# EarthyScience/EasyHybrid.jl

Hardware: AMD Instinct MI355X
Metric: training samples/sec (higher is better)
Workload: dtype f32; 1 GPU; RbQ10 hybrid, MLP [2,16,16,1] tanh -> rb (sigmoid-scaled), Q10 global, MSE + Adam(0.01), batch=65536 per GPU, fp32 (BASELINE.json configs[1]); global_batch=65536, resident_batches_per_gpu=64, parallelism=dp1, ranks_seen=1, launcher=none, gradient_exchange=none (one GPU)

## Files before the change

### easyhybrid.jl_amd/csrc/eh_api.hip

```cpp
#include <hip/hip_runtime.h>
#include <chrono>

#include <algorithm>
#include <cfloat>
#include <atomic>
#include <cmath>
#include <cstdarg>
#include <cstdio>
#include <cstdlib>
#include <cstring>
#include <memory>
#include <mutex>
#include <string>
#include <thread>
#include <vector>

#include "eh_internal.hpp"
#include "eh_kernels.hpp"
#include "eh_chain.hpp"
#include "eh_lbfgs.hpp"
#include "eh_wide.hpp"
#include "eh_seq.hpp"

std::string g_create_err;
// ... 794 lines not shown
    if (!(h->own_stream = stream_pool_take(h->device))) HIPCHK_C(hipStreamCreateWithFlags(&h->own_stream, hipStreamNonBlocking));
    tick("stream");
    h->stream = h->own_stream;
    for (int vi = 0; vi < arch->nvar; ++vi) HIPCHK_C(arch->var[vi].prepare());
    tick("kernel attributes");
    if (const char* ej = getenv("EH_JIT")) h->jit_on = atoi(ej) != 0;
    if (const char* es = getenv("EH_SPECIALIZE")) h->specialize = atoi(es) != 0;
    if (getenv("EH_NO_AOT_SPEC")) h->aot_spec = false;
    if (d->mech == EH_MECH_PROGRAM) {
        std::vector<unsigned> pb(EH_PROG_HDR + EH_MAX_PROG, 0u);
        pb[0] = (unsigned)d->prog_len; pb[1] = (unsigned)d->prog_n_out;
        for (int o = 0; o < EH_MAX_PROG_OUT; ++o) pb[2 + o] = (unsigned)(o < d->prog_n_out ? d->prog_out[o] : d->prog_out[0]);
        for (int k = 0; k < d->prog_n_const; ++k) memcpy(&pb[8 + k], &d->prog_const[k], sizeof(float));
        for (int i = 0; i < d->prog_len; ++i) pb[EH_PROG_HDR + i] = d->prog_code[i];
        HIPCHK_C(hipMalloc(&h->prog, pb.size() * sizeof(unsigned)));
        HIPCHK_C(hipMemcpy(h->prog, pb.data(), pb.size() * sizeof(unsigned), hipMemcpyHostToDevice));
    }
    const size_t nt = (size_t)n.n_theta;
    HIPCHK_C(hipMalloc(&h->pset, (6 * nt + 4 * EH_MAX_OPT_GROUPS) * sizeof(float)));
    HIPCHK_C(hipMemset(h->pset, 0, (6 * nt + 4 * EH_MAX_OPT_GROUPS) * sizeof(float)));
    for (int k = 0; k < 2; ++k) { h->thb[k] = h->pset + (size_t)k * 3 * nt; h->mb[k] = h->thb[k] + nt; h->vb[k] = h->thb[k] + 2 * nt; }
    h->sc = h->pset + 6 * nt;
    h->bn_on = d->input_batchnorm != 0;
    if (h->bn_on) {
        HIPCHK_C(hipMalloc(&h->bn_part, (32 * 64 + 32) * sizeof(float)));
        HIPCHK_C(hipMalloc(&h->bn_run, 64 * sizeof(float)));
        HIPCHK_C(hipMalloc(&h->bn_shift, 32 * sizeof(float)));
        HIPCHK_C(hipMemset(h->bn_shift, 0, 32 * sizeof(float)));
        HIPCHK_C(hipMalloc(&h->bn_stat, 68 * sizeof(float)));
        HIPCHK_C(hipMemset(h->bn_stat, 0, 68 * sizeof(float)));
        float run0[64];
        for (int p = 0; p < 32; ++p) { run0[p] = 0.0f; run0[32 + p] = 1.0f; }
        HIPCHK_C(hipMemcpy(h->bn_run, run0, sizeof run0, hipMemcpyHostToDevice));
    }
    if (h->bnl) {
        const int tot = h->bnl_maxn;
        int widest = 0;
        for (int l = 0; l < h->l_net[0].nl; ++l) if (h->l_net[0].lbn[l]) widest = std::max(widest, h->l_net[0].out[l]);
        h->bnl_maxn = widest;
        std::vector<float> run0((size_t)tot, 0.0f);
        for (int l = 0; l < h->l_net[0].nl; ++l)
            if (h->l_net[0].lbn[l]) std::fill(run0.begin() + h->bnl_off[l] + h->l_net[0].out[l], run0.begin() + h->bnl_off[l] + 2 * h->l_net[0].out[l], 1.0f);
        HIPCHK_C(hipMalloc(&h->bnl_run, (size_t)tot * sizeof(float)));
        HIPCHK_C(hipMemcpy(h->bnl_run, run0.data(), (size_t)tot * sizeof(float), hipMemcpyHostToDevice));
        HIPCHK_C(hipMalloc(&h->bnl_stat, (size_t)2 * tot * sizeof(float)));
        HIPCHK_C(hipMemset(h->bnl_stat, 0, (size_t)2 * tot * sizeof(float)));
        HIPCHK_C(hipMalloc(&h->bnl_part, (size_t)(EH_BNL_CHUNKS + 1) * 2 * widest * sizeof(float)));
    }
    if (!lform && !seq) {
        HIPCHK_C(hipMalloc(&h->gacc, ((size_t)3 * EH_GSHARDS * h->n_acc + 4) * sizeof(float)));
        HIPCHK_C(hipMemset(h->gacc, 0, ((size_t)3 * EH_GSHARDS * h->n_acc + 4) * sizeof(float)));
        h->ord_soff = (n.n_theta + 3) & ~3;
        h->ord_rs = h->ord_soff + ((h->n_acc - n.n_theta + 3) & ~3);
        const size_t ob = sizeof(unsigned) * 32 * EH_ORD_GROUPS + sizeof(float) * (size_t)2 * (EH_ORD_ROWS + EH_ORD_GROUPS) * h->ord_rs;
        HIPCHK_C(hipMalloc(&h->ord, ob));
        HIPCHK_C(hipMemset(h->ord, 0, ob));
        HIPCHK_C(hipMemsetD32(reinterpret_cast<hipDeviceptr_t>(h->ord + 32 * EH_ORD_GROUPS), (int)EH_ORD_EMPTY, (size_t)2 * EH_ORD_ROWS * h->ord_rs));
        HIPCHK_C(hipHostMalloc((void**)&h->ord_err, sizeof(unsigned), hipHostMallocMapped));
        *h->ord_err = 0u;
    }
    tick("pset / bn / gacc");
    h->slab_rows = lform ? (int)EH_LFORM_ROWS : h->max_blocks;
    HIPCHK_C(hipMalloc(&h->slab, (std::max((size_t)h->slab_rows * std::max(h->n_acc, EH_EVAL_STATS * n.T), (size_t)1 << 20) + 16) * sizeof(float)));
    HIPCHK_C(hipMalloc(&h->gradbuf, (size_t)h->n_acc * sizeof(float)));
    HIPCHK_C(hipMalloc(&h->mombuf, EH_MAX_TARG * EH_EVAL_STATS * sizeof(float)));
    HIPCHK_C(hipMemset(h->mombuf, 0, EH_MAX_TARG * EH_EVAL_STATS * sizeof(float)));
    HIPCHK_C(hipMalloc(&h->tcount, 3 * EH_MAX_TARG * sizeof(float)));
    HIPCHK_C(hipMemset(h->tcount, 0, 3 * EH_MAX_TARG * sizeof(float)));
    HIPCHK_C(hipMalloc(&h->inv_n, EH_TT * EH_MAX_TARG * sizeof(float)));
    HIPCHK_C(hipMemset(h->inv_n, 0, EH_TT * EH_MAX_TARG * sizeof(float)));
    HIPCHK_C(hipMemset(h->gradbuf, 0, (size_t)h->n_acc * sizeof(float)));
    tick("slab + small buffers");
    if (seq) {
        std::vector<unsigned char> wf((size_t)n.n_theta, 0);
        const int* o = h->seq_off;
        std::fill(wf.begin() + o[EH_SEQ_WIN], wf.begin() + o[EH_SEQ_BIN], (unsigned char)1);
        std::fill(wf.begin() + o[EH_SEQ_WHD], wf.begin() + o[EH_SEQ_BHD], (unsigned char)1);
        std::fill(wf.begin() + o[EH_SEQ_WOUT], wf.begin() + o[EH_SEQ_BOUT], (unsigned char)1);
        HIPCHK_C(hipMalloc(&h->wflag, wf.size()));
        HIPCHK_C(hipMemcpy(h->wflag, wf.data(), wf.size(), hipMemcpyHostToDevice));
    }
    else if (!lform) { if (int rc = build_maps(h, true)) { g_create_err = h->err; eh_destroy(h); return rc; } }
    else {
        std::vector<unsigned char> wf((size_t)n.n_theta, 0);
        for (int k = 0; k < h->l_nnets; ++k)
            for (int l = 0; l < h->l_net[k].nl; ++l)
                if (!h->l_net[k].lbn[l]) std::fill(wf.begin() + h->l_net[k].woff[l], wf.begin() + h->l_net[k].boff[l], (unsigned char)1);
        HIPCHK_C(hipMalloc(&h->wflag, wf.size()));
        HIPCHK_C(hipMemcpy(h->wflag, wf.data(), wf.size(), hipMemcpyHostToDevice));
    }
    tick("maps");
    {
        std::vector<float> img0((size_t)arch->img_floats, 0.0f);
        for (int j = 0; j < d->n_params; ++j) {
            if (d->param_kind[j] == EH_PAR_FIXED) img0[arch->phi_off + EH_IMG_PHI + j] = d->param_default[j];
            img0[arch->phi_off + EH_IMG_LO + j] = d->param_lower[j];
            img0[arch->phi_off + EH_IMG_SC + j] = d->param_upper[j] - d->param_lower[j];
        }
        for (int p = 0; p < 32; ++p) { img0[arch->phi_off + EH_IMG_BNM + p] = 0.0f; img0[arch->phi_off + EH_IMG_BNR + p] = d->input_batchnorm ? 1.0f / std::sqrt(1.0f + EH_BN_EPS) : 1.0f; }
        for (int k = 0; k < (lform ? 0 : n_nets); ++k)
            for (int l = net_d[k]; l < nl; ++l)
                for (int i = 0; i < net_w[k][l]; ++i)
                    img0[arch->wh_off + (size_t)(l - 1) * arch->hp * arch->sh + (size_t)(h->net_r0[k][l] + i) * arch->sh + h->net_r0[k][l - 1] + i] = 1.0f;
        auto put_int = [&](int slot, int v) { memcpy(&img0[arch->phi_off + slot], &v, sizeof(int)); };
        if (!lform && !seq) {
            for (int l = 0; l <= d->n_hidden; ++l) { put_int(EH_IMG_WOFF + l, lw_off[l]); put_int(EH_IMG_BOFF + l, lb_off[l]); }
            for (int l = 0; l < d->n_hidden; ++l) put_int(EH_IMG_WIDTH + l, tot_w[l]);
// ... 707 lines not shown
    if (!spec_lookup(h) && jit_wanted(h, EH_MODE_TRAIN)) {
        eh_handle_s::JitEntry* je = jit_entry(const_cast<eh_handle*>(h));
        if (je && (!je->verified || !je->k.fn[EH_MODE_TRAIN_MULTI])) return false;
    }
    return true;
}
static int do_fused_multi(eh_handle* h, const EhSplit& sp, const int* idx, long long first, long long batch, long long end, int nsteps, float* loss_slots) {
    if (h->pending && h->pend_ord) FLUSH(h);
    EhStepArgs a = eh_step_args(h, sp, idx, first, std::min(batch, end - first));
    a.image = h->image; a.slab = h->slab; a.n_acc = h->n_acc; a.inv_n = nullptr; a.rmap = h->rmap; a.stamps = h->stamps;
    EhFused& z = a.fz;
    z.gacc = h->gacc; z.pset = h->pset; z.imap = h->imap; z.loss_slot = h->pending_loss;
    z.gslot = (int)(h->gstep % 3); z.cur = h->cur; z.sc_sel = h->sc_sel; z.pending = h->pending ? 1 : 0; z.opt = h->opt; z.agg_a = h->img.agg_a;
    a.p2p = nullptr; a.p2p_seq = 0u;
    if (int rc = eh_bn_prepare(h, sp, idx, first, a.count, true, &a)) return rc;
    a.ms_nsteps = nsteps; a.ms_batch = (int)batch; a.ms_end = end; a.ms_loss = loss_slots;
    HIPCHK(h, step_launch(h, EH_MODE_TRAIN_MULTI, 1, &a));
    h->cur ^= 1; h->sc_sel ^= 1;
    h->gstep += 1;
    h->pending = false;
    h->pending_loss = nullptr;
    return EH_OK;
}

static int launch_chain(eh_handle* h, bool raw, float* sc_in, float* sc_out, float* loss_slot) {
    static const int one_env = getenv("EH_CHAIN_ONE") ? atoi(getenv("EH_CHAIN_ONE")) : -1;
    const int nt = h->net.n_theta;
    const bool l2 = raw && (h->img.l2c != 0.0f || h->img.l2w);
    const unsigned tp = raw ? two_pass_mask(h->net) : 0u;
    const EhChainSrc src{raw ? 1 : 0, h->net.loss, h->net.T, tp, tp ? h->inv_n : nullptr, l2 ? h->l2val : nullptr};
    unsigned long long* ctr = reinterpret_cast<unsigned long long*>(h->chain_part + EH_CHAIN_PARTS);
    if (h->chain.i_norm < 0) {
        hipLaunchKernelGGL(eh_chain_apply_kernel<false>, dim3((nt + 255) / 256), dim3(256), 0, h->stream, h->gradbuf, nt, TH(h), MM(h), VV(h), sc_in, sc_out, h->opt,
                           h->chain, src, h->img, h->chain_part, 0, loss_slot, ctr);
    } else if (nt <= (one_env >= 0 ? one_env : (int)EH_CHAIN_ONE_MAX)) {
        hipLaunchKernelGGL(eh_chain_apply_kernel<true>, dim3(1), dim3(256), 0, h->stream, h->gradbuf, nt, TH(h), MM(h), VV(h), sc_in, sc_out, h->opt,
                           h->chain, src, h->img, h->chain_part, 0, loss_slot, ctr);
    } else {
        const int nb = std::min<int>(EH_CHAIN_PARTS, (nt + 1023) / 1024);
        hipLaunchKernelGGL(eh_chain_norm_kernel, dim3(nb), dim3(256), 0, h->stream, h->gradbuf, nt, TH(h), h->chain, src, h->img, h->chain_part);
        HIPCHK(h, hipGetLastError());
        hipLaunchKernelGGL(eh_chain_apply_kernel<false>, dim3((nt + 255) / 256), dim3(256), 0, h->stream, h->gradbuf, nt, TH(h), MM(h), VV(h), sc_in, sc_out, h->opt,
                           h->chain, src, h->img, h->chain_part, nb, loss_slot, ctr);
    }
    HIPCHK(h, hipGetLastError());
    return EH_OK;
}

static bool ord_ok(const eh_handle* h, int grid) {
    static const int cw_env = getenv("EH_REDUCE_CW") ? atoi(getenv("EH_REDUCE_CW")) : 0;
    if (!h->fused || !h->fused_det || !h->ord || grid <= 1 || grid > (int)EH_ORD_ROWS || h->chain.n || h->drop_on) return false;
    if (h->lform || h->arch->wide || h->p2p_on || h->net.T != 1 || h->net.mech == EH_MECH_PROGRAM || h->net.loss == EH_LOSS_PROGRAM || h->act == EH_ACT_PER_NET) return false;
    if (h->img.l2c != 0.0f || h->img.l2w || two_pass_mask(h->net) || h->dp_weights || h->dp_moments) return false;
    return h->n_acc < 8192 && h->ord_rs <= h->arch->img_floats && (cw_env == 0 || cw_env == 16);
}

int eh_do_step(eh_handle* h, const EhSplit& sp, const int* idx, long long first, long long count, bool apply, bool raw, float* loss_slot) {
    const EhNet& net = h->net;
    EhProf prof;
    if (int rc = prof_begin(h, &prof)) return rc;
    int grid = 1;
    const int deferred = (net.T == 1 && !raw) ? 1 : 0;
    const unsigned tp_mask = two_pass_mask(net);
    const bool moment_loss = tp_mask != 0;
    const bool l2 = (h->img.l2c != 0.0f || h->img.l2w) && !raw;
    float* sc_in = h->sc + 2 * h->sc_sel;
    float* sc_out = h->sc + 2 * (h->sc_sel ^ 1);
    EhLApply lap{};
    h->l_apply = nullptr; h->l_applied = false;
    const bool chained = apply && h->chain.n != 0;
    if (h->lform && apply && deferred && !l2 && !moment_loss && net.loss != EH_LOSS_PROGRAM) {
        lap.theta = TH(h); lap.m = MM(h); lap.v = VV(h); lap.sc_in = sc_in; lap.sc_out = sc_out; lap.o = h->opt; lap.loss_slot = loss_slot; lap.gradbuf = h->gradbuf;
        lap.im = h->img; lap.loss_kind = h->net.loss; lap.n_theta = net.n_theta; lap.g_off = net.g_off;
        if (chained) {
            HIPCHK(h, hipMemsetAsync(h->gradbuf, 0, (size_t)net.n_theta * sizeof(float), h->stream));
            lap.theta = h->gradbuf;
            lap.o = EhOpt{EH_OPT_DESCENT, -1.0f, 1.0f, 1.0f, 0.0f, 0.0f, nullptr};
            lap.im.g_off = net.n_theta; lap.im.imap = nullptr;
        }
        h->l_apply = &lap;
    }
    int rc = launch_train_kernel(h, sp, idx, first, count, &grid, apply);
    h->l_apply = nullptr;
    if (rc) return rc;
    if (h->drop_on && apply) h->drop_step++;
    const bool mid = prof.on && !prof.burst;
    if (mid) HIPCHK(h, hipEventRecord(h->ev[h->ev_used + 1], h->stream));
    if (h->l_applied) {
        h->l_applied = false;
        if (chained) {
            if (int rcc = launch_chain(h, false, sc_in, sc_out, nullptr)) return rcc;
        }
        h->sc_sel ^= 1;
        return prof_end(h, prof, mid);
    }
    if (l2) {
        hipLaunchKernelGGL(eh_weight_l2_kernel, dim3(1), dim3(256), 0, h->stream, TH(h), h->img, h->l2val);
        HIPCHK(h, hipGetLastError());
    }
    static const int cw_env = getenv("EH_REDUCE_CW") ? atoi(getenv("EH_REDUCE_CW")) : 0;
    const bool big = cw_env ? cw_env == 64 : h->n_acc >= 8192;
    const bool tall = cw_env ? cw_env == 256 : (h->lform && grid <= (int)EH_LFORM_ROWS && h->n_acc >= 16384);
    static const bool nc1 = getenv("EH_REDUCE_NC1") != nullptr;
    const bool tall4 = tall && !nc1;
    const int rgrid = tall4 ? (h->n_acc + 1023) / 1024 : tall ? (h->n_acc + 255) / 256 : big ? (h->n_acc + 63) / 64 : (h->n_acc + 15) / 16;
#define EH_REDUCE_GO(AP, ...)                                                                                                                       \
// ... 967 lines not shown
```

### easyhybrid.jl_amd/csrc/eh_device.hpp

```cpp
#pragma once
#ifndef __HIPCC_RTC__
#include <hip/hip_runtime.h>
#include <stdint.h>
#endif

#include "easyhybrid_hip.h"

#define EH_BN_SELF_MAX 512
#define EH_EVAL_STATS 8

typedef float f32x4 __attribute__((ext_vector_type(4)));

enum { EH_MODE_TRAIN = 0, EH_MODE_EVAL = 1, EH_MODE_TRAIN_P2P = 2, EH_MODE_TRAIN_MULTI = 3, EH_MODE_TRAIN_ORD = 4 };

struct EhNet {
    int P, K, G, T, F;
    int n_theta, g_off;
    int scale_nn, mech, n_par;
    int loss;
    int n_out;
    unsigned targ_out;
    unsigned par_kind;
    unsigned par_idx;
    unsigned forc_col;
// ... 32 lines not shown
    } else if (o.rule == EH_OPT_RMSPROP) {
        v = o.b1 * v + (1.0f - o.b1) * (g * g);
        th -= g * (o.lr / (sqrtf(v) + o.eps));
    } else {
        th -= o.lr * g;
    }
}

template <class PB>
__device__ __forceinline__ void eh_opt_update_at(const EhOpt& o, PB bt, long long i, float g, float bt1, float bt2, float& th, float& m, float& v) {
    if (o.tab == nullptr) { eh_opt_update(o, g, bt1, bt2, th, m, v); return; }
    const int k = o.tab->gid[i];
    eh_opt_update(o.tab->r[k], g, bt[4 * k], bt[4 * k + 1], th, m, v);
}
template <class PI, class PO>
__device__ __forceinline__ void eh_opt_advance_groups(const EhOptTab* tab, PI bt_in, PO bt_out, bool upd) {
    const int n = tab->n;
    for (int k = 0; k < n; ++k) {
        const float p1 = bt_in[4 * k], p2 = bt_in[4 * k + 1];
        bt_out[4 * k] = upd ? p1 * tab->r[k].b1 : p1;
        bt_out[4 * k + 1] = upd ? p2 * tab->r[k].b2 : p2;
    }
}

__device__ __forceinline__ void eh_loss_finish(int kind, float S, float n, float Sy, float Syy, float& scale, float& loss, float agg = 1.0f) {
    if (!(n > 0.0f)) { scale = 0.0f; loss = __builtin_nanf(""); return; }
    if (kind == EH_LOSS_RMSE) {
        loss = sqrtf(S / n);
        scale = 1.0f / (2.0f * n * loss);
    } else if (kind == EH_LOSS_NSELOSS) {
        const float D = Syy - Sy * Sy / n;
        loss = S / D;
        scale = 1.0f / D;
    } else {
        scale = 1.0f / n;
        loss = S * scale;
    }
    if (agg != 1.0f) { scale *= agg; loss *= agg; }
}

#define EH_GSHARDS 8

struct EhP2P {
    unsigned long long* peer_recv[EH_GSHARDS];
    float* stage;
    unsigned* counter;
    int* err;
    int world, rank;
    int mode;
};

template <int CTRL> __device__ __forceinline__ float eh_dpp(float v);
enum { EH_ORD_GROUPS = 16, EH_ORD_ROWS = 256 };
struct EhOrd {
    float* rows;
    float* grows;
    unsigned* cnt;
    unsigned* err;
    int rs, soff;
    int slot;
    int prev_grid;
};
#define EH_ORD_EMPTY 0x7FA5A5A5u
#define EH_ORD_DEADLINE_TICKS 200000000ull
enum { EH_ORD_ST_TAIL = 32, EH_ORD_ST_PRO = EH_ORD_ST_TAIL + 10 * EH_ORD_GROUPS, EH_STAMP_WORDS = 256 };
#ifdef EH_STAMPS
#define EH_ORD_TICK(ts, p)                                                                            \
    do {                                                                                               \
        __builtin_amdgcn_sched_barrier(0);                                                             \
        ts[2 * (p)] = __builtin_readcyclecounter(); ts[2 * (p) + 1] = wall_clock64();                  \
        __builtin_amdgcn_sched_barrier(0);                                                             \
    } while (0)
#else
#define EH_ORD_TICK(ts, p)
#endif
__device__ __forceinline__ int eh_ord_pos(int e, int nth, int soff) { return e < nth ? e : soff + (e - nth); }
#ifdef EH_AB_ORD_PARENT
__device__ __forceinline__ int eh_ord_scalar_row(int lane) { return lane; }
__device__ __forceinline__ f32x4 eh_ord_scalar_fold(const EhOrd& o, int lane, const f32x4 (&v)[4]) {
    float w[4][4];
#pragma unroll
    for (int j = 0; j < 4; ++j)
#pragma unroll
        for (int k = 0; k < 4; ++k) {
            float c = 0.0f;
            if (lane + 64 * j < o.prev_grid) c += v[j][k];
#pragma unroll
            for (int off = 32; off >= 1; off >>= 1) c += __shfl_xor(c, off, 64);
            w[j][k] = c;
        }
    f32x4 t;
#pragma unroll
    for (int k = 0; k < 4; ++k) t[k] = (w[0][k] + w[1][k]) + (w[2][k] + w[3][k]);
    return t;
}
#else
__device__ __forceinline__ int eh_ord_scalar_row(int lane) { return 4 * (lane & ~15) + (lane & 15); }
__device__ __forceinline__ f32x4 eh_ord_scalar_fold(const EhOrd& o, int lane, const f32x4 (&v)[4]) {
    const int r0 = eh_ord_scalar_row(lane);
    f32x4 t;
#pragma unroll
    for (int k = 0; k < 4; ++k) {
        float c[4];
#pragma unroll
        for (int j = 0; j < 4; ++j) {
            c[j] = 0.0f;
            if (r0 + 16 * j < o.prev_grid) c[j] += v[j][k];
        }
        float s = (c[0] + c[2]) + (c[1] + c[3]);
        s += eh_dpp<0x128>(s);
        s += eh_dpp<0x124>(s);
        s += eh_dpp<0x4E>(s);
        s += eh_dpp<0xB1>(s);
        const int si = __builtin_bit_cast(int, s);
        const float w0 = __builtin_bit_cast(float, __builtin_amdgcn_readlane(si, 0)), w1 = __builtin_bit_cast(float, __builtin_amdgcn_readlane(si, 16)),
                    w2 = __builtin_bit_cast(float, __builtin_amdgcn_readlane(si, 32)), w3 = __builtin_bit_cast(float, __builtin_amdgcn_readlane(si, 48));
        t[k] = (w0 + w1) + (w2 + w3);
    }
    return t;
}
#endif
__device__ __forceinline__ void eh_ord_scalar_loads(const EhOrd& o, int lane, f32x4 (&v)[4]) {
    const float* const R = o.rows + (long long)(o.slot ^ 1) * EH_ORD_ROWS * o.rs + o.soff;
    const int r0 = eh_ord_scalar_row(lane);
#pragma unroll
    for (int j = 0; j < 4; ++j) {
        const int r = r0 + 16 * j;
        v[j] = r < o.prev_grid ? *(const f32x4*)(R + (long long)r * o.rs) : f32x4{0.0f, 0.0f, 0.0f, 0.0f};
    }
}
__device__ __forceinline__ void eh_ord_group_loads(const EhOrd& o, int idx, float (&g)[EH_ORD_GROUPS]) {
    const float* const G = o.grows + (long long)(o.slot ^ 1) * EH_ORD_GROUPS * o.rs + idx;
#pragma unroll
    for (int k = 0; k < EH_ORD_GROUPS; ++k) g[k] = k < o.prev_grid ? G[(long long)k * o.rs] : 0.0f;
}
__device__ __forceinline__ float eh_ord_group_fold(const float (&g)[EH_ORD_GROUPS]) {
    float t = 0.0f;
#pragma unroll
    for (int k = 0; k < EH_ORD_GROUPS; ++k) t += g[k];
    return t;
}
typedef unsigned u32x4_ord __attribute__((ext_vector_type(4)));
__device__ __forceinline__ __amdgpu_buffer_rsrc_t eh_ord_rsrc(const float* base, int nfloats) {
    return __builtin_amdgcn_make_buffer_rsrc(const_cast<float*>(base), (short)0, 4 * nfloats, 0x00020000);
}
__device__ __forceinline__ f32x4 eh_ord_ld16(__amdgpu_buffer_rsrc_t r, int off) { return __builtin_bit_cast(f32x4, __builtin_amdgcn_raw_buffer_load_b128(r, off, 0, 16)); }
__device__ __forceinline__ void eh_ord_st16(__amdgpu_buffer_rsrc_t r, int off, f32x4 v) { __builtin_amdgcn_raw_buffer_store_b128(__builtin_bit_cast(u32x4_ord, v), r, off, 0, 16); }
enum { EH_ORD_OOB = 0x7FFFFFF0 };
__device__ __forceinline__ void eh_ord_reset(const EhOrd& o, int b, int nblk, int tid, int nthr) {
    const __amdgpu_buffer_rsrc_t rr = eh_ord_rsrc(o.rows, 2 * EH_ORD_ROWS * o.rs);
    const float e = __uint_as_float(EH_ORD_EMPTY);
    const f32x4 ev = {e, e, e, e};
    const int nv = o.soff >> 2;
    for (int r = b; r < o.prev_grid; r += nblk)
        for (int v = tid; v < nv; v += nthr) eh_ord_st16(rr, 4 * (((o.slot ^ 1) * EH_ORD_ROWS + r) * o.rs) + 16 * v, ev);
}
__device__ __forceinline__ void eh_ord_publish(const EhOrd& o, int nth, int tid, int nthr, const float* row, float* flag, unsigned long long* st) {
#ifdef EH_STAMPS
    unsigned long long ts[10];
#endif
    EH_ORD_TICK(ts, 0);
    const unsigned gi = blockIdx.x % EH_ORD_GROUPS, gsz = (gridDim.x - gi + EH_ORD_GROUPS - 1) / EH_ORD_GROUPS;
    const __amdgpu_buffer_rsrc_t rr = eh_ord_rsrc(o.rows, 2 * EH_ORD_ROWS * o.rs);
    const int nv = (nth + 3) >> 2;
#ifdef EH_AB_ORD_PARENT
    asm volatile("s_waitcnt vmcnt(0)" ::: "memory");
#endif
    __syncthreads();
    if (__builtin_amdgcn_readfirstlane(tid >> 6) == 0) {
        const int rb = 4 * ((o.slot * EH_ORD_ROWS + (int)blockIdx.x) * o.rs);
        for (int v = tid; v <= nv; v += 64) {
            const int w = v < nv ? 4 * v : o.soff;
            eh_ord_st16(rr, rb + 4 * w, *(const f32x4*)&row[w]);
        }
        EH_ORD_TICK(ts, 1);
        if (tid == 0) {
            unsigned* const gc = o.cnt + 32 * gi;
            const bool last = __hip_atomic_fetch_add(gc, 1u, __ATOMIC_RELAXED, __HIP_MEMORY_SCOPE_AGENT) == gsz - 1;
            if (last) __hip_atomic_store(gc, 0u, __ATOMIC_RELAXED, __HIP_MEMORY_SCOPE_AGENT);
            flag[0] = last ? 1.0f : 0.0f;
        }
    }
    __syncthreads();
    EH_ORD_TICK(ts, 2);
    if (flag[0] == 0.0f) return;
    constexpr int NK = EH_ORD_ROWS / EH_ORD_GROUPS;
    const int kown = blockIdx.x / EH_ORD_GROUPS;
    const int rb = 4 * ((o.slot * EH_ORD_ROWS + (int)gi) * o.rs), rk = 4 * EH_ORD_GROUPS * o.rs;
    const __amdgpu_buffer_rsrc_t gr = eh_ord_rsrc(o.grows, 2 * EH_ORD_GROUPS * o.rs);
    const int gb = 4 * ((o.slot * EH_ORD_GROUPS + (int)gi) * o.rs);
    for (int v = tid; v < nv; v += nthr) {
        f32x4 r[NK];
#pragma unroll
        for (int k = 0; k < NK; ++k) r[k] = eh_ord_ld16(rr, ((unsigned)k < gsz && k != kown) ? rb + k * rk + 16 * v : (int)EH_ORD_OOB);
        const f32x4 own = *(const f32x4*)&row[4 * v];
        auto fold = [&]() {
            f32x4 s = {0.0f, 0.0f, 0.0f, 0.0f};
#pragma unroll
            for (int k = 0; k < NK; ++k) s += k == kown ? own : r[k];
            return s;
        };
        f32x4 s = fold();
        bool nan = false;
#pragma unroll
        for (int j = 0; j < 4; ++j) nan = nan || (4 * v + j < nth && s[j] != s[j]);
        if (nan) {
            auto empty = [&](int k) {
                bool e = false;
#pragma unroll
                for (int j = 0; j < 4; ++j) e = e || (4 * v + j < nth && __float_as_uint(r[k][j]) == EH_ORD_EMPTY);
                return e;
            };
            bool in = true;
#pragma unroll
            for (int k = 0; k < NK; ++k) in = in && !empty(k);
            if (!in) {
                const unsigned long long t0 = wall_clock64();
                bool late = false;
                s = f32x4{0.0f, 0.0f, 0.0f, 0.0f};
#pragma unroll 1
                for (int k = 0; k < NK; ++k) {
                    f32x4 q = own;
                    if (k != kown) {
                        const int off = (unsigned)k < gsz ? rb + k * rk + 16 * v : (int)EH_ORD_OOB;
                        auto empty_q = [&]() {
                            bool e = false;
#pragma unroll
                            for (int j = 0; j < 4; ++j) e = e || (4 * v + j < nth && __float_as_uint(q[j]) == EH_ORD_EMPTY);
                            return e;
                        };
                        q = eh_ord_ld16(rr, off);
                        while (!late && empty_q()) {
                            if (wall_clock64() - t0 > EH_ORD_DEADLINE_TICKS) { __hip_atomic_store(o.err, 1u, __ATOMIC_RELAXED, __HIP_MEMORY_SCOPE_SYSTEM); late = true; break; }
                            __builtin_amdgcn_s_sleep(1);
                            q = eh_ord_ld16(rr, off);
                        }
                    }
                    s += q;
                }
            }
        }
        eh_ord_st16(gr, gb + 16 * v, s);
    }
// ... 698 lines not shown
    int nx_glb = 0;
    bool nx_live = false;
    auto fetch_idx = [&](int tile) {
        const int n_loc = tile * MT + lane;
        nx_live = (tile < ntiles) && (lane < MT) && (n_loc < count);
        nx_glb = nx_live ? (a.idx ? a.idx[first + n_loc] : first + n_loc) : 0;
    };
    auto fetch_rec_into = [&](EhRec<NX4>& dst) {
        const bool live = nx_live;
        const float* const rec = a.recs + (long long)nx_glb * a.C;
        if ((a.C & 3) == 0) {
#pragma unroll
            for (int q = 0; q < NX4; ++q) dst.x[q] = (live && 4 * q < net.P) ? *(const f32x4*)(rec + 4 * q) : f32x4{0, 0, 0, 0};
        } else {
#pragma unroll
            for (int q = 0; q < NX4; ++q)
#pragma unroll
                for (int e = 0; e < 4; ++e) dst.x[q][e] = (live && 4 * q + e < net.P) ? rec[4 * q + e] : 0.0f;
        }
#pragma unroll
        for (int f = 0; f < EH_MAX_FORC; ++f) dst.frc[f] = (fCol[f] >= 0 && live) ? rec[fCol[f]] : 0.0f;
#pragma unroll
        for (int t = 0; t < EH_MAX_TARG; ++t) dst.y[t] = (tOn[t] != 0.0f && live) ? rec[tcol0 + t] : __builtin_nanf("");
    };
    auto fetch_rec = [&]() { fetch_rec_into(nx); };
    auto fetch = [&](int tile) { fetch_idx(tile); fetch_rec(); };
    const bool carried = carry && carry->valid;
    bool rec_pending = false;
    if (carried) { nx = carry->rec; nx_live = carry->live; }
    else {
        fetch_idx((int)blockIdx.x * NW + wave);
        rec_pending = a.idx != nullptr;
        if (!rec_pending) fetch_rec();
    }
    bool pf_issued = false;

    EH_STAMP(0);
    const bool fusedm = TRAIN && a.fz.gacc != nullptr;
    float f_th = 0.0f, f_m = 0.0f, f_v = 0.0f, f_g = 0.0f, f_cnt = 0.0f, f_sse = 0.0f, f_sy = 0.0f, f_syy = 0.0f, f_bt1 = 0.0f, f_bt2 = 0.0f;
    int f_map = 0;
    int f_rcode = 0;
    if constexpr (TRAIN) f_rcode = (a.rmap && tid < a.n_acc) ? a.rmap[tid] : 0;
    float f_rm = 0.0f, f_rv = 0.0f;
    if ((a.bn_part || a.bn_nblk == -1) && a.bn_update && blockIdx.x == 0 && tid < net.P) { f_rm = a.bn_run[tid]; f_rv = a.bn_run[32 + tid]; }
    const bool deferred_upd = fusedm && !(a.ms_direct && a.ms_keep);
    const int px_mode = P2PM ? a.p2pv.mode : 0, px_rank = P2PM ? a.p2pv.rank : 0, px_world = P2PM ? a.p2pv.world : 1;
    const unsigned long long* const px_recv = P2PM ? a.p2pv.peer_recv[px_rank] + (long long)((a.fz.gslot + 2) % 3) * EH_GSHARDS * a.n_acc : nullptr;
    const float* const px_stage = P2PM ? a.p2pv.stage : nullptr;
    float px_own[5] = {0.0f, 0.0f, 0.0f, 0.0f, 0.0f};
    const bool own_direct = deferred_upd && a.fz.pending && (!P2PM || px_mode == 1);
    float f_sv = 0.0f;
    float f_gs[EH_GSHARDS] = {0.0f, 0.0f, 0.0f, 0.0f, 0.0f, 0.0f, 0.0f, 0.0f};
    float o_g[ORDM ? EH_ORD_GROUPS : 1];
    f32x4 o_sv[ORDM ? 4 : 1];
    if constexpr (ORDM) {
#pragma unroll
        for (int k = 0; k < EH_ORD_GROUPS; ++k) o_g[k] = 0.0f;
#pragma unroll
        for (int j = 0; j < 4; ++j) o_sv[j] = f32x4{0.0f, 0.0f, 0.0f, 0.0f};
    }
    if (deferred_upd) {
        const EhFused& z = a.fz;
        const float* const g_prev = (P2PM ? px_stage : z.gacc) + ((z.gslot + 2) % 3) * (EH_GSHARDS * a.n_acc);
        const float* const pin = z.pset + z.cur * 3 * net.n_theta;
        if constexpr (ORDM) { if (own_direct && wave == 0) eh_ord_scalar_loads(a.ord, lane, o_sv); }
        else { if (own_direct && lane < 40) f_sv = g_prev[(lane & 7) * a.n_acc + net.n_theta + (lane >> 3)]; }
        const float* const sc_in = z.pset + 6 * net.n_theta + 2 * z.sc_sel;
        f_bt1 = sc_in[0]; f_bt2 = sc_in[1];
        if (tid < net.n_theta) {
            f_th = pin[tid]; f_m = pin[net.n_theta + tid]; f_v = pin[2 * net.n_theta + tid];
            f_map = tid < net.g_off ? z.imap[tid] : 0;
            if (own_direct) {
                if constexpr (ORDM) eh_ord_group_loads(a.ord, tid, o_g);
                else {
#pragma unroll
                    for (int sh = 0; sh < EH_GSHARDS; ++sh) f_gs[sh] = g_prev[sh * a.n_acc + tid];
                }
            }
        }
    }
    EH_STAMP_PRO(2);
    float* const px_T = eh_px_table<P2PM || ORDM>();
    const int px_nmain = net.n_theta < NTHR ? net.n_theta : NTHR;
    const unsigned px_seq = a.p2p_seq - 1u;
    const unsigned long long px_none = (unsigned long long)px_seq << 32;
    unsigned long long px_w[P2PM ? EH_GSHARDS : 1], px_s[P2PM ? EH_GSHARDS : 1];
    const int px_k = tid - (NTHR - 8);
    const bool px_sc = px_k >= 0 && px_k < (net.T > 3 ? 5 : 4);
    auto px_request = [&]() {
#pragma unroll
        for (int sh = 0; sh < (P2PM ? EH_GSHARDS : 1); ++sh) {
            px_w[sh] = px_none; px_s[sh] = px_none;
            if (sh < px_world && !(px_mode == 1 && sh == px_rank)) {
                const unsigned long long* const q = px_recv + (long long)sh * a.n_acc;
                if (tid < px_nmain) px_w[sh] = __hip_atomic_load(q + tid, __ATOMIC_RELAXED, __HIP_MEMORY_SCOPE_SYSTEM);
                if (px_sc) px_s[sh] = __hip_atomic_load(q + net.n_theta + px_k, __ATOMIC_RELAXED, __HIP_MEMORY_SCOPE_SYSTEM);
            }
        }
    };
    if constexpr (P2PM) {
        if (fusedm && a.fz.pending && px_mode == 1 && px_world > 1 && blockIdx.x == 0) eh_p2p_fold_store(&a.p2pv, (a.fz.gslot + 2) % 3, px_seq, a.n_acc, tid, NTHR, true);
        if (fusedm && a.fz.pending) px_request();
    }
    EH_STAMP_PRO(3);
    if (!a.ms_keep) {
        constexpr int NI = (G::IMG_FLOATS / 4 + NTHR - 1) / NTHR, NIB = NI < 16 ? NI : 16;
        for (int e0 = 4 * tid; e0 < G::IMG_FLOATS; e0 += 4 * NTHR * NIB) {
            f32x4 tmp[NIB];
#pragma unroll
            for (int u = 0; u < NIB; ++u) {
                const int e = e0 + 4 * NTHR * u;
                tmp[u] = e < G::IMG_FLOATS ? *(const f32x4*)&a.image[e] : f32x4{0, 0, 0, 0};
            }
            if (rec_pending) { fetch_rec(); rec_pending = false; }
#pragma unroll
            for (int u = 0; u < NIB; ++u) {
                const int e = e0 + 4 * NTHR * u;
                if (e < G::IMG_FLOATS) *(f32x4*)&wl[e] = tmp[u];
            }
        }
    }
    if (rec_pending) fetch_rec();
    if (ORDM && own_direct) {
        if constexpr (ORDM) {
#ifdef EH_STAMPS
            if (a.stamps && blockIdx.x == 0 && tid == 0) { unsigned long long ts[4]; EH_ORD_TICK(ts, 0); a.stamps[EH_ORD_ST_PRO] = ts[0]; a.stamps[EH_ORD_ST_PRO + 1] = ts[1]; }
#endif
            f_g = eh_ord_group_fold(o_g);
            if (wave == 0) {
                const f32x4 t = eh_ord_scalar_fold(a.ord, lane, o_sv);
                if (lane == 0) *(f32x4*)px_T = t;
#ifdef EH_STAMPS
                if (a.stamps && blockIdx.x == 0 && tid == 0) { unsigned long long ts[4]; EH_ORD_TICK(ts, 1); a.stamps[EH_ORD_ST_PRO + 2] = ts[2]; a.stamps[EH_ORD_ST_PRO + 3] = ts[3]; }
#endif
            }
        }
    } else if (own_direct) {
        f_g = eh_fold8(f_gs[0], f_gs[1], f_gs[2], f_gs[3], f_gs[4], f_gs[5], f_gs[6], f_gs[7]);
        const int svi = __builtin_bit_cast(int, eh_fold8_lanes(f_sv));
        const float S0 = __builtin_bit_cast(float, __builtin_amdgcn_readlane(svi, 0)), S1 = __builtin_bit_cast(float, __builtin_amdgcn_readlane(svi, 8)),
                    S2 = __builtin_bit_cast(float, __builtin_amdgcn_readlane(svi, 16)), S3 = __builtin_bit_cast(float, __builtin_amdgcn_readlane(svi, 24)),
                    S4 = __builtin_bit_cast(float, __builtin_amdgcn_readlane(svi, 32));
        if constexpr (P2PM) { px_own[0] = S0; px_own[1] = S1; px_own[2] = S2; px_own[3] = S3; px_own[4] = S4; }
        else {
            f_sse = S0; f_cnt = S1 + (net.T > 1 ? S2 : 0.0f) + (net.T > 2 ? S3 : 0.0f) + (net.T > 3 ? S4 : 0.0f); f_sy = S2; f_syy = S3;
        }
    }
    EH_STAMP_PRO(4);
    if constexpr (P2PM) {
        if (fusedm && a.fz.pending) {
            {
                unsigned long long t0 = 0;
                bool timing = false;
                while (true) {
                    bool all = true;
#pragma unroll
                    for (int sh = 0; sh < EH_GSHARDS; ++sh)
                        if (sh < px_world) all = all && ((unsigned)(px_w[sh] >> 32) == px_seq) && ((unsigned)(px_s[sh] >> 32) == px_seq);
                    if (all) break;
                    if (__hip_atomic_load(a.p2pv.err, __ATOMIC_RELAXED, __HIP_MEMORY_SCOPE_AGENT)) break;
                    if (!timing) { t0 = wall_clock64(); timing = true; }
                    else if (wall_clock64() - t0 > EH_P2P_DEADLINE_TICKS) { __hip_atomic_store(a.p2pv.err, 1, __ATOMIC_RELAXED, __HIP_MEMORY_SCOPE_AGENT); break; }
                    __builtin_amdgcn_s_sleep(2);
                    px_request();
                }
            }
            EH_STAMP_PRO(11);
            const bool own1 = px_mode == 1;
            const float own_g = f_g;
            const float own_s = px_k == 0 ? px_own[0] : px_k == 1 ? px_own[1] : px_k == 2 ? px_own[2] : px_k == 3 ? px_own[3] : px_own[4];
            float fs = 0.0f;
            f_g = 0.0f;
#pragma unroll
            for (int sh = 0; sh < EH_GSHARDS; ++sh)
                if (sh < px_world) {
                    const bool own = own1 && sh == px_rank;
                    f_g += own ? own_g : ((unsigned)(px_w[sh] >> 32) == px_seq) ? __uint_as_float((unsigned)px_w[sh]) : 0.0f;
                    fs += own ? own_s : ((unsigned)(px_s[sh] >> 32) == px_seq) ? __uint_as_float((unsigned)px_s[sh]) : 0.0f;
                }
            if (px_k >= 0) px_T[px_k] = fs;
            EH_STAMP_PRO(12);
            __syncthreads();
            EH_STAMP_PRO(13);
            {
                const f32x4 t4 = *(const f32x4*)px_T;
                f_sse = t4[0];
// ... 1095 lines not shown
```

### easyhybrid.jl_amd/csrc/eh_kernels.hpp

```cpp
#pragma once
#include "eh_internal.hpp"

__global__ __launch_bounds__(256) void eh_weight_l2_kernel(const float* theta, EhImg im, float* out) {
    __shared__ float red[4];
    float s = 0.0f;
    if (im.l2w) {
        for (int i = threadIdx.x; i < im.n_theta; i += 256) { const float w = theta[i]; s = fmaf(im.l2w[i] * w, w, s); }
    } else {
        for (int i = threadIdx.x; i < im.g_off; i += 256)
            if (eh_is_weight(im, i)) { const float w = theta[i]; s += w * w; }
    }
#pragma unroll
    for (int o = 32; o >= 1; o >>= 1) s += __shfl_xor(s, o, 64);
    if ((threadIdx.x & 63) == 0) red[threadIdx.x >> 6] = s;
    __syncthreads();
    if (threadIdx.x == 0) *out = im.l2s * (im.l2w ? 1.0f : im.l2c) * ((red[0] + red[1]) + (red[2] + red[3]));
}

__global__ void eh_image_kernel(const float* theta, int n_theta, EhImg im) {
    const int idx = blockIdx.x * blockDim.x + threadIdx.x;
    if (idx < n_theta) eh_image_store(im, idx, theta[idx]);
}


// ... 234 lines not shown
        float got[6 * EH_GSHARDS];
        eh_ll_issue(ad, seq, w);
        eh_ll_finish(p2p, ad, seq, w, got);
        float s1 = 0.0f, s2 = 0.0f, s3 = 0.0f, s4 = 0.0f;
#pragma unroll
        for (int sh = 0; sh < EH_GSHARDS; ++sh) {
            const bool me = own_direct && sh == p2p->rank;
            sse += me ? ownv[0] : got[6 * sh]; s1 += me ? ownv[1] : got[6 * sh + 1]; s2 += me ? ownv[2] : got[6 * sh + 2];
            s3 += me ? ownv[3] : got[6 * sh + 3]; s4 += me ? ownv[4] : got[6 * sh + 4]; gs_p2p += me ? ownv[5] : got[6 * sh + 5];
        }
        cnt = s1 + (T > 1 ? s2 : 0.0f) + (T > 2 ? s3 : 0.0f) + (T > 3 ? s4 : 0.0f); sy = s2; syy = s3;
    } else {
        static_assert(EH_GSHARDS == 8, "eh_fold8");
        float S[5] = {0.0f, 0.0f, 0.0f, 0.0f, 0.0f};
#pragma unroll
        for (int k = 0; k < 5; ++k) {
            if (k == 4 && T <= 3) continue;
            const float* q = g_prev + n_theta + k;
            S[k] = eh_fold8(q[0], q[n_acc], q[2 * n_acc], q[3 * n_acc], q[4 * n_acc], q[5 * n_acc], q[6 * n_acc], q[7 * n_acc]);
        }
        sse = S[0]; cnt = S[1] + (T > 1 ? S[2] : 0.0f) + (T > 2 ? S[3] : 0.0f) + (T > 3 ? S[4] : 0.0f); sy = S[2]; syy = S[3];
    }
    float inv = 0.0f, lossv = 0.0f;
    if (T == 1) eh_loss_finish(loss_kind, sse, cnt, sy, syy, inv, lossv, im.agg_a);
    else { inv = cnt > 0.0f ? 1.0f : 0.0f; lossv = cnt > 0.0f ? sse : __builtin_nanf(""); }
    float th = th0;
    if (own && cnt > 0.0f) {
        const float gs = p2p ? gs_p2p : eh_fold8(gsv[0], gsv[1], gsv[2], gsv[3], gsv[4], gsv[5], gsv[6], gsv[7]);
        float mm = mm0, vv = vv0;
        eh_opt_update_at(o, sc_in, idx, gs * inv, sc0, sc1, th, mm, vv);
        theta[idx] = th; m[idx] = mm; v[idx] = vv;
    }
    if (own) {
        if (idx < im.g_off) { if (mp0 >= 0) im.image[mp0] = th; }
        else eh_image_store(im, idx, th);
    }
    if (idx == 0) {
        if (o.tab) eh_opt_advance_groups(o.tab, sc_in, sc_out, cnt > 0.0f);
        else {
            sc_out[0] = cnt > 0.0f ? sc0 * o.b1 : sc0;
            sc_out[1] = cnt > 0.0f ? sc1 * o.b2 : sc1;
        }
        if (loss_slot) *loss_slot = lossv;
    }
}

__global__ __launch_bounds__(256) void eh_ord_flush_kernel(const EhOrd o, int n_theta, float* theta, float* m, float* v, const float* sc_in, float* sc_out,
                                                           EhOpt op, float* loss_slot, EhImg im, int loss_kind) {
    eh_ord_reset(o, blockIdx.x, gridDim.x, threadIdx.x, 256);
    if ((int)blockIdx.x * 256 >= n_theta) return;
    const int idx = blockIdx.x * 256 + threadIdx.x, lane = threadIdx.x & 63;
    const bool own = idx < n_theta;
    float gv[EH_ORD_GROUPS];
    f32x4 sv[4];
    eh_ord_group_loads(o, own ? idx : 0, gv);
    eh_ord_scalar_loads(o, lane, sv);
    float th = 0.0f, mm = 0.0f, vv = 0.0f;
    int mp = -1;
    if (own) { th = theta[idx]; mm = m[idx]; vv = v[idx]; if (idx < im.g_off && im.imap) mp = im.imap[idx]; }
    const float bt1 = sc_in[0], bt2 = sc_in[1];
    const f32x4 t = eh_ord_scalar_fold(o, lane, sv);
    float inv = 1.0f, lossv = 0.0f;
    eh_loss_finish(loss_kind, t[0], t[1], t[2], t[3], inv, lossv, im.agg_a);
    const bool upd = t[1] > 0.0f;
    if (own && upd) {
        eh_opt_update_at(op, sc_in, idx, eh_ord_group_fold(gv) * inv, bt1, bt2, th, mm, vv);
        theta[idx] = th; m[idx] = mm; v[idx] = vv;
    }
    if (own) {
        if (idx < im.g_off) { if (mp >= 0) im.image[mp] = th; }
        else eh_image_store(im, idx, th);
    }
    if (idx == 0) {
        if (op.tab) eh_opt_advance_groups(op.tab, sc_in, sc_out, upd);
        else {
            sc_out[0] = upd ? bt1 * op.b1 : bt1;
            sc_out[1] = upd ? bt2 * op.b2 : bt2;
        }
        if (loss_slot) *loss_slot = upd ? lossv + 0.0f : __builtin_nanf("");
    }
}

__device__ __forceinline__ bool eh_kind_two_pass(unsigned kind, int T) {
    return (kind >= (unsigned)EH_LOSS_PEARSONLOSS && kind <= (unsigned)EH_LOSS_PBKGELOSS) || (kind == (unsigned)EH_LOSS_RMSE && T > 1);
}
__global__ __launch_bounds__(64) void eh_moment_centre_kernel(const float* slab, int nblk, int T, unsigned loss_t, EhShift4 shift, float* tt) {
    __shared__ double tot[EH_EVAL_STATS];
    const int tid = threadIdx.x, t = blockIdx.x;
    if (!eh_kind_two_pass((loss_t >> (4 * t)) & 15u, T)) return;
    if (tid < EH_EVAL_STATS) {
        double s = 0.0;
        for (int b = 0; b < nblk; ++b) s += (double)slab[(b * T + t) * EH_EVAL_STATS + tid];
        tot[tid] = s;
    }
    __syncthreads();
    if (tid == 0) tt[EH_TT * t + 1] = tot[3] > 0.0 ? (float)((double)shift.c[t] + tot[4] / tot[3]) : shift.c[t];
}
__global__ __launch_bounds__(64) void eh_moment_coef_kernel(const float* slab, int nblk, int T, unsigned loss_t, EhShift4 shift4, float* tt_all, float agg_a) {
    __shared__ double tot[EH_EVAL_STATS];
    const int tid = threadIdx.x, t = blockIdx.x;
    const int kind = (int)((loss_t >> (4 * t)) & 15u);
    if (!eh_kind_two_pass((unsigned)kind, T)) return;
    float* const out = tt_all + EH_TT * t;
    const float shift = shift4.c[t];
    if (tid < EH_EVAL_STATS) {
        double s = 0.0;
        for (int b = 0; b < nblk; ++b) s += (double)slab[(b * T + t) * EH_EVAL_STATS + tid];
// ... 190 lines not shown
```

Before: 6.377 billion samples/s.

## Pre-reduce ordered loss scalars per group into a partial buffer

Adds a small per-group partial buffer where the last wave of each group-reducing block pre-folds the four loss scalars across its rows, waiting on empty sentinels if needed. The next step's prologue and flush kernel then load one f32x4 per lane from this buffer instead of four row loads, and fold with DPP and readlane. The work can run on the last wave when the parameter count leaves it idle. It adds a spin-wait path and restricts the ordered mode to layouts with exactly four scalar slots.

```diff
diff --git a/easyhybrid.jl_amd/csrc/eh_api.hip b/easyhybrid.jl_amd/csrc/eh_api.hip
--- a/easyhybrid.jl_amd/csrc/eh_api.hip
+++ b/easyhybrid.jl_amd/csrc/eh_api.hip
@@ -870,7 +870,7 @@
         HIPCHK_C(hipMemset(h->gacc, 0, ((size_t)3 * EH_GSHARDS * h->n_acc + 4) * sizeof(float)));
         h->ord_soff = (n.n_theta + 3) & ~3;
         h->ord_rs = h->ord_soff + ((h->n_acc - n.n_theta + 3) & ~3);
-        const size_t ob = sizeof(unsigned) * 32 * EH_ORD_GROUPS + sizeof(float) * (size_t)2 * (EH_ORD_ROWS + EH_ORD_GROUPS) * h->ord_rs;
+        const size_t ob = sizeof(unsigned) * 32 * EH_ORD_GROUPS + sizeof(float) * ((size_t)2 * (EH_ORD_ROWS + EH_ORD_GROUPS) * h->ord_rs + 2 * EH_ORD_PART);
         HIPCHK_C(hipMalloc(&h->ord, ob));
         HIPCHK_C(hipMemset(h->ord, 0, ob));
         HIPCHK_C(hipMemsetD32(reinterpret_cast<hipDeviceptr_t>(h->ord + 32 * EH_ORD_GROUPS), (int)EH_ORD_EMPTY, (size_t)2 * EH_ORD_ROWS * h->ord_rs));
@@ -1684,6 +1684,7 @@
     if (!h->fused || !h->fused_det || !h->ord || grid <= 1 || grid > (int)EH_ORD_ROWS || h->chain.n || h->drop_on) return false;
     if (h->lform || h->arch->wide || h->p2p_on || h->net.T != 1 || h->net.mech == EH_MECH_PROGRAM || h->net.loss == EH_LOSS_PROGRAM || h->act == EH_ACT_PER_NET) return false;
     if (h->img.l2c != 0.0f || h->img.l2w || two_pass_mask(h->net) || h->dp_weights || h->dp_moments) return false;
+    if (h->n_acc != h->net.n_theta + 4 || h->ord_rs != h->ord_soff + 4) return false;
     return h->n_acc < 8192 && h->ord_rs <= h->arch->img_floats && (cw_env == 0 || cw_env == 16);
 }
 
diff --git a/easyhybrid.jl_amd/csrc/eh_device.hpp b/easyhybrid.jl_amd/csrc/eh_device.hpp
--- a/easyhybrid.jl_amd/csrc/eh_device.hpp
+++ b/easyhybrid.jl_amd/csrc/eh_device.hpp
@@ -108,6 +108,10 @@
 
 template <int CTRL> __device__ __forceinline__ float eh_dpp(float v);
 enum { EH_ORD_GROUPS = 16, EH_ORD_ROWS = 256 };
+enum { EH_ORD_PART = 4 * EH_ORD_GROUPS * 4 };
+#if defined(EH_AB_ORD_PARENT) && !defined(EH_AB_ORD_ROW_SCALARS)
+#define EH_AB_ORD_ROW_SCALARS
+#endif
 struct EhOrd {
     float* rows;
     float* grows;
@@ -131,6 +135,30 @@
 #define EH_ORD_TICK(ts, p)
 #endif
 __device__ __forceinline__ int eh_ord_pos(int e, int nth, int soff) { return e < nth ? e : soff + (e - nth); }
+#ifndef EH_AB_ORD_ROW_SCALARS
+enum { EH_ORD_NSV = 1 };
+__device__ __forceinline__ f32x4 eh_ord_scalar_fold(const EhOrd& o, int lane, const f32x4 (&v)[EH_ORD_NSV]) {
+    f32x4 t;
+#pragma unroll
+    for (int k = 0; k < 4; ++k) {
+        float s = v[0][k];
+        s += eh_dpp<0x128>(s);
+        s += eh_dpp<0x124>(s);
+        s += eh_dpp<0x4E>(s);
+        s += eh_dpp<0xB1>(s);
+        const int si = __builtin_bit_cast(int, s);
+        const float w0 = __builtin_bit_cast(float, __builtin_amdgcn_readlane(si, 0)), w1 = __builtin_bit_cast(float, __builtin_amdgcn_readlane(si, 16)),
+                    w2 = __builtin_bit_cast(float, __builtin_amdgcn_readlane(si, 32)), w3 = __builtin_bit_cast(float, __builtin_amdgcn_readlane(si, 48));
+        t[k] = (w0 + w1) + (w2 + w3);
+    }
+    return t;
+}
+__device__ __forceinline__ void eh_ord_scalar_loads(const EhOrd& o, int lane, f32x4 (&v)[EH_ORD_NSV]) {
+    const float* const P = o.grows + (long long)2 * EH_ORD_GROUPS * o.rs + (o.slot ^ 1) * EH_ORD_PART + 4 * lane;
+    v[0] = (lane & (EH_ORD_GROUPS - 1)) < o.prev_grid ? *(const f32x4*)P : f32x4{0.0f, 0.0f, 0.0f, 0.0f};
+}
+#else
+enum { EH_ORD_NSV = 4 };
 #ifdef EH_AB_ORD_PARENT
 __device__ __forceinline__ int eh_ord_scalar_row(int lane) { return lane; }
 __device__ __forceinline__ f32x4 eh_ord_scalar_fold(const EhOrd& o, int lane, const f32x4 (&v)[4]) {
@@ -185,6 +213,7 @@
         v[j] = r < o.prev_grid ? *(const f32x4*)(R + (long long)r * o.rs) : f32x4{0.0f, 0.0f, 0.0f, 0.0f};
     }
 }
+#endif
 __device__ __forceinline__ void eh_ord_group_loads(const EhOrd& o, int idx, float (&g)[EH_ORD_GROUPS]) {
     const float* const G = o.grows + (long long)(o.slot ^ 1) * EH_ORD_GROUPS * o.rs + idx;
 #pragma unroll
@@ -207,7 +236,11 @@
     const __amdgpu_buffer_rsrc_t rr = eh_ord_rsrc(o.rows, 2 * EH_ORD_ROWS * o.rs);
     const float e = __uint_as_float(EH_ORD_EMPTY);
     const f32x4 ev = {e, e, e, e};
+#ifdef EH_AB_ORD_ROW_SCALARS
     const int nv = o.soff >> 2;
+#else
+    const int nv = (o.soff >> 2) + 1;
+#endif
     for (int r = b; r < o.prev_grid; r += nblk)
         for (int v = tid; v < nv; v += nthr) eh_ord_st16(rr, 4 * (((o.slot ^ 1) * EH_ORD_ROWS + r) * o.rs) + 16 * v, ev);
 }
@@ -243,8 +276,46 @@
     constexpr int NK = EH_ORD_ROWS / EH_ORD_GROUPS;
     const int kown = blockIdx.x / EH_ORD_GROUPS;
     const int rb = 4 * ((o.slot * EH_ORD_ROWS + (int)gi) * o.rs), rk = 4 * EH_ORD_GROUPS * o.rs;
-    const __amdgpu_buffer_rsrc_t gr = eh_ord_rsrc(o.grows, 2 * EH_ORD_GROUPS * o.rs);
+    const __amdgpu_buffer_rsrc_t gr = eh_ord_rsrc(o.grows, 2 * EH_ORD_GROUPS * o.rs + 2 * EH_ORD_PART);
     const int gb = 4 * ((o.slot * EH_ORD_GROUPS + (int)gi) * o.rs);
+    const int pb = 4 * (2 * EH_ORD_GROUPS * o.rs + o.slot * EH_ORD_PART + 4 * (int)gi), pq = 4 * 4 * EH_ORD_GROUPS;
+    if (__builtin_amdgcn_readfirstlane(tid >> 6) == (nthr >> 6) - 1) {
+        const int k = tid & 63;
+        const int off = ((unsigned)k < gsz && k != kown) ? rb + k * rk + 4 * o.soff : (int)EH_ORD_OOB;
+        f32x4 q = eh_ord_ld16(rr, off);
+        if (k == kown) q = *(const f32x4*)&row[o.soff];
+        auto blocks = [&]() {
+            f32x4 c = f32x4{0.0f, 0.0f, 0.0f, 0.0f} + q;
+#pragma unroll
+            for (int j = 0; j < 4; ++j) {
+                float s = c[j];
+                s += eh_dpp<0x4E>(s);
+                s += eh_dpp<0xB1>(s);
+                c[j] = s;
+            }
+            return c;
+        };
+        f32x4 p = blocks();
+        bool nan = false;
+#pragma unroll
+        for (int j = 0; j < 4; ++j) nan = nan || p[j] != p[j];
+        if (__builtin_amdgcn_ballot_w64(nan) != 0ull) {
+            auto empty_q = [&]() {
+                bool e = false;
+#pragma unroll
+                for (int j = 0; j < 4; ++j) e = e || __float_as_uint(q[j]) == EH_ORD_EMPTY;
+                return e;
+            };
+            const unsigned long long t0 = wall_clock64();
+            while (empty_q()) {
+                if (wall_clock64() - t0 > EH_ORD_DEADLINE_TICKS) { __hip_atomic_store(o.err, 1u, __ATOMIC_RELAXED, __HIP_MEMORY_SCOPE_SYSTEM); break; }
+                __builtin_amdgcn_s_sleep(1);
+                q = eh_ord_ld16(rr, off);
+            }
+            p = blocks();
+        }
+        if (k < EH_ORD_GROUPS && (k & 3) == 0) eh_ord_st16(gr, pb + (k >> 2) * pq, p);
+    }
     for (int v = tid; v < nv; v += nthr) {
         f32x4 r[NK];
 #pragma unroll
@@ -1049,18 +1120,23 @@
     float f_sv = 0.0f;
     float f_gs[EH_GSHARDS] = {0.0f, 0.0f, 0.0f, 0.0f, 0.0f, 0.0f, 0.0f, 0.0f};
     float o_g[ORDM ? EH_ORD_GROUPS : 1];
-    f32x4 o_sv[ORDM ? 4 : 1];
+    f32x4 o_sv[ORDM ? EH_ORD_NSV : 1];
+#if defined(EH_AB_ORD_ROW_SCALARS) || defined(EH_AB_ORD_FOLD_WAVE0)
+    const int o_wave = 0;
+#else
+    const int o_wave = (ORDM && net.n_theta <= NTHR - 64) ? NTHR / 64 - 1 : 0;
+#endif
     if constexpr (ORDM) {
 #pragma unroll
         for (int k = 0; k < EH_ORD_GROUPS; ++k) o_g[k] = 0.0f;
 #pragma unroll
-        for (int j = 0; j < 4; ++j) o_sv[j] = f32x4{0.0f, 0.0f, 0.0f, 0.0f};
+        for (int j = 0; j < EH_ORD_NSV; ++j) o_sv[j] = f32x4{0.0f, 0.0f, 0.0f, 0.0f};
     }
     if (deferred_upd) {
         const EhFused& z = a.fz;
         const float* const g_prev = (P2PM ? px_stage : z.gacc) + ((z.gslot + 2) % 3) * (EH_GSHARDS * a.n_acc);
         const float* const pin = z.pset + z.cur * 3 * net.n_theta;
-        if constexpr (ORDM) { if (own_direct && wave == 0) eh_ord_scalar_loads(a.ord, lane, o_sv); }
+        if constexpr (ORDM) { if (own_direct && wave == o_wave) eh_ord_scalar_loads(a.ord, lane, o_sv); }
         else { if (own_direct && lane < 40) f_sv = g_prev[(lane & 7) * a.n_acc + net.n_theta + (lane >> 3)]; }
         const float* const sc_in = z.pset + 6 * net.n_theta + 2 * z.sc_sel;
         f_bt1 = sc_in[0]; f_bt2 = sc_in[1];
@@ -1121,14 +1197,14 @@
     if (ORDM && own_direct) {
         if constexpr (ORDM) {
 #ifdef EH_STAMPS
-            if (a.stamps && blockIdx.x == 0 && tid == 0) { unsigned long long ts[4]; EH_ORD_TICK(ts, 0); a.stamps[EH_ORD_ST_PRO] = ts[0]; a.stamps[EH_ORD_ST_PRO + 1] = ts[1]; }
+            if (a.stamps && blockIdx.x == 0 && wave == o_wave && lane == 0) { unsigned long long ts[4]; EH_ORD_TICK(ts, 0); a.stamps[EH_ORD_ST_PRO] = ts[0]; a.stamps[EH_ORD_ST_PRO + 1] = ts[1]; }
 #endif
             f_g = eh_ord_group_fold(o_g);
-            if (wave == 0) {
+            if (wave == o_wave) {
                 const f32x4 t = eh_ord_scalar_fold(a.ord, lane, o_sv);
                 if (lane == 0) *(f32x4*)px_T = t;
 #ifdef EH_STAMPS
-                if (a.stamps && blockIdx.x == 0 && tid == 0) { unsigned long long ts[4]; EH_ORD_TICK(ts, 1); a.stamps[EH_ORD_ST_PRO + 2] = ts[2]; a.stamps[EH_ORD_ST_PRO + 3] = ts[3]; }
+                if (a.stamps && blockIdx.x == 0 && lane == 0) { unsigned long long ts[4]; EH_ORD_TICK(ts, 1); a.stamps[EH_ORD_ST_PRO + 2] = ts[2]; a.stamps[EH_ORD_ST_PRO + 3] = ts[3]; }
 #endif
             }
         }
diff --git a/easyhybrid.jl_amd/csrc/eh_kernels.hpp b/easyhybrid.jl_amd/csrc/eh_kernels.hpp
--- a/easyhybrid.jl_amd/csrc/eh_kernels.hpp
+++ b/easyhybrid.jl_amd/csrc/eh_kernels.hpp
@@ -310,7 +310,7 @@
     const int idx = blockIdx.x * 256 + threadIdx.x, lane = threadIdx.x & 63;
     const bool own = idx < n_theta;
     float gv[EH_ORD_GROUPS];
-    f32x4 sv[4];
+    f32x4 sv[EH_ORD_NSV];
     eh_ord_group_loads(o, own ? idx : 0, gv);
     eh_ord_scalar_loads(o, lane, sv);
     float th = 0.0f, mm = 0.0f, vv = 0.0f;
```

Measured after the change: 6.746 billion samples/s (median of 6 runs). 5.8% higher.
